# hzyu17/GaussianVI

Measured on AMD Instinct MI355X. Metric: sigma-point psi-evals/sec + NGD iters/sec, 1024-factor d=12 p=5 chain, higher is better.
Workload: dtype f64; 1 GPU; c3: T=1025 states, n=6; 1 step = 1 device-resident NGD iteration; restart every 30; factor_sets_columns=[K factors, d, GH degree p, N sigma points], factor_set_kinds=1024 x quadratic-prior d=12 p=5 (N=17217); 1025 x fixed-prior d=6 p=5 (N=1433), kernel_variant=6, chunks_per_factor=4, fused_pass=True, one_launch_factor_stage=False, mirror_pairs=False, fuse_trial=2

## Files before the change

### gaussianvi_amd/_lib.py

```python
from __future__ import annotations

import ctypes as C
import os

HERE = os.path.dirname(os.path.abspath(__file__))
LIB_PATH = os.environ.get("GVI_LIB_PATH") or os.path.join(HERE, "libgvi_hip.so")

c_double_p = C.POINTER(C.c_double)
c_int32_p = C.POINTER(C.c_int32)
c_int8_p = C.POINTER(C.c_int8)
c_void_pp = C.POINTER(C.c_void_p)
ALLGATHER_FN = C.CFUNCTYPE(C.c_int, C.c_void_p, C.c_void_p, C.c_void_p, C.c_int64, C.c_void_p)

SIGNATURES = {
    "gvi_ctx_create": [C.c_int, C.c_int, c_void_pp],
    "gvi_ctx_destroy": [C.c_void_p],
    "gvi_ctx_set_stream": [C.c_void_p, C.c_void_p],
    "gvi_ctx_sync": [C.c_void_p],
    "gvi_spgh_count": [C.c_int, C.c_int, C.POINTER(C.c_int64)],
    "gvi_spgh_nodes": [C.c_int, C.c_int, C.c_int64, C.c_void_p, C.c_void_p, C.c_void_p],
    "gvi_chain_set": [C.c_void_p, C.c_int, C.c_int],
    "gvi_factors_add": [C.c_void_p, C.c_int, C.c_int, C.c_int, C.c_void_p, C.c_int, C.c_void_p, C.c_int64,
                        C.c_void_p, C.POINTER(C.c_int)],
    "gvi_factors_add_table": [C.c_void_p, C.c_int, C.c_int, C.c_int, C.c_void_p, C.c_int, C.c_void_p, C.c_int64,
# ... 16 lines not shown
    "gvi_prox_step": [C.c_void_p, C.c_double, C.c_int, C.c_void_p, C.c_void_p, C.c_void_p, C.c_void_p],
    "gvi_factors_set_closed_form": [C.c_void_p, C.c_int, C.c_int],
    "gvi_factors_set_sdf3d": [C.c_void_p, C.c_int, C.c_void_p, C.c_double, C.c_int, C.c_int, C.c_int, C.c_void_p],
    "gvi_factors_set_arm": [C.c_void_p, C.c_int, C.c_int, C.c_void_p, C.c_void_p, C.c_void_p, C.c_void_p, C.c_int, C.c_void_p,
                            C.c_void_p, C.c_void_p],
    "gvi_factors_set_temperature": [C.c_void_p, C.c_int, C.c_void_p],
    "gvi_factors_info": [C.c_void_p, C.c_int, C.POINTER(C.c_int), C.POINTER(C.c_int), C.POINTER(C.c_int),
                         C.POINTER(C.c_int64)],
    "gvi_moments": [C.c_void_p, C.c_int] + [C.c_void_p] * 5,
    "gvi_moments_dev": [C.c_void_p, C.c_int] + [C.c_void_p] * 5,
    "gvi_raw_moments": [C.c_void_p, C.c_int] + [C.c_void_p] * 5,
    "gvi_costs": [C.c_void_p, C.c_int] + [C.c_void_p] * 3,
    "gvi_costs_dev": [C.c_void_p, C.c_int] + [C.c_void_p] * 3,
    "gvi_expand": [C.c_void_p, C.c_int] + [C.c_void_p] * 3,
    "gvi_moments_from_psi": [C.c_void_p, C.c_int] + [C.c_void_p] * 6,
    "gvi_bt_assemble": [C.c_void_p, C.c_int, C.c_void_p, C.c_void_p, C.c_void_p, C.c_void_p, C.c_void_p, C.c_void_p],
    "gvi_bt_solve": [C.c_void_p] + [C.c_void_p] * 4,
    "gvi_bt_logdet": [C.c_void_p] + [C.c_void_p] * 3,
    "gvi_bt_marginals": [C.c_void_p] + [C.c_void_p] * 4,
    "gvi_gather_marginals": [C.c_void_p, C.c_int] + [C.c_void_p] * 5,
    "gvi_ngd_init": [C.c_void_p] + [C.c_void_p] * 3,
    "gvi_ngd_cost": [C.c_void_p, c_double_p],
    "gvi_ngd_factor_costs": [C.c_void_p, C.c_int, C.c_void_p],
    "gvi_ngd_gradients": [C.c_void_p],
    "gvi_ngd_trial": [C.c_void_p, C.c_double, c_double_p],
    "gvi_ngd_accept": [C.c_void_p],
    "gvi_ngd_step": [C.c_void_p, C.c_double, C.c_int, c_double_p, C.POINTER(C.c_int), c_double_p, C.POINTER(C.c_int)],
    "gvi_ngd_run": [C.c_void_p, C.c_int, C.c_double, C.c_int, C.c_void_p, C.c_void_p, C.c_void_p, C.c_void_p, C.POINTER(C.c_int)],
    "gvi_ngd_set_mode": [C.c_void_p, C.c_int, C.c_int],
    "gvi_ngd_counters": [C.c_void_p, C.POINTER(C.c_int64), C.POINTER(C.c_int64), C.c_int],
    "gvi_ngd_gradients_local": [C.c_void_p],
    "gvi_ngd_gradients_finish": [C.c_void_p],
    "gvi_ngd_cost_local": [C.c_void_p],
    "gvi_ngd_cost_finish": [C.c_void_p, c_double_p],
    "gvi_ngd_trial_local": [C.c_void_p, C.c_double],
    "gvi_ngd_trial_finish": [C.c_void_p, c_double_p],
    "gvi_ngd_exchange": [C.c_void_p, C.c_int, c_void_pp, C.POINTER(C.c_int64)],
    "gvi_dist_unique_id": [C.c_void_p],
    "gvi_dist_init_rccl": [C.c_void_p, C.c_int, C.c_int, C.c_void_p],
    "gvi_dist_init_callback": [C.c_void_p, C.c_int, C.c_int, C.c_void_p, C.c_void_p],
    "gvi_dist_info": [C.c_void_p, C.POINTER(C.c_int), C.POINTER(C.c_int), C.POINTER(C.c_int)],
    "gvi_ngd_get_state": [C.c_void_p] + [C.c_void_p] * 5,
    "gvi_ngd_get_gradients": [C.c_void_p] + [C.c_void_p] * 6,
    "gvi_randn": [C.c_void_p, C.c_uint64, C.c_int64, C.c_int64, C.c_void_p],
    "gvi_bt_sample": [C.c_void_p, C.c_void_p, C.c_void_p, C.c_void_p, C.c_int, C.c_uint64, C.c_int64, C.c_void_p, C.c_void_p],
    "gvi_ngd_sample": [C.c_void_p, C.c_int, C.c_uint64, C.c_int64, C.c_void_p],
# ... 47 lines not shown
```

### gaussianvi_amd/api.py

```python
from __future__ import annotations

import ctypes as C

import numpy as np

from . import _lib

PSI_RANGE_1D, PSI_QUAD_PRIOR, PSI_FIXED_PRIOR, PSI_HOST_CALLBACK, PSI_HINGE_SDF_2D = 0, 1, 2, 3, 4
PSI_HINGE_SDF_2D_BODY, PSI_HINGE_SDF_3D, PSI_HINGE_SDF_3D_ARM = 5, 6, 7
RULE_NGD, RULE_PROX_JKO = 0, 1
GVI_F64, GVI_F32 = 0, 1


class GviError(RuntimeError):
    def __init__(self, status, msg):
        super().__init__(f"gvi status {status}: {msg}")
        self.status = status


def _f64(a):
    return np.ascontiguousarray(a, dtype=np.float64)


def _p(a):
# ... 212 lines not shown
        return SD, SU

    def gather_marginals(self, sid, mu, SigD, SigU):
        K, d, _, _ = self.sets[sid]
        mu, SigD, SigU = _f64(mu), _f64(SigD), _f64(SigU)
        mk, Sk = np.empty((K, d)), np.empty((K, d, d))
        self._ck(self.lib.gvi_gather_marginals(self.h, sid, _p(mu), _p(SigD), _p(SigU), _p(mk), _p(Sk)))
        return mk, Sk

    def ngd_init(self, mu, D, U):
        mu, D, U = _f64(mu), _f64(D), _f64(U)
        self._ck(self.lib.gvi_ngd_init(self.h, _p(mu), _p(D), _p(U)))

    def ngd_cost(self):
        v = C.c_double()
        self._ck(self.lib.gvi_ngd_cost(self.h, C.byref(v)))
        return v.value

    def ngd_factor_costs(self, sid):
        out = np.empty(self.sets[sid][0])
        self._ck(self.lib.gvi_ngd_factor_costs(self.h, sid, _p(out)))
        return out

    def ngd_gradients(self):
        self._ck(self.lib.gvi_ngd_gradients(self.h))

    def ngd_gradients_local(self):
        self._ck(self.lib.gvi_ngd_gradients_local(self.h))

    def ngd_gradients_finish(self):
        self._ck(self.lib.gvi_ngd_gradients_finish(self.h))

    def ngd_cost_local(self):
        self._ck(self.lib.gvi_ngd_cost_local(self.h))

    def ngd_cost_finish(self):
        v = C.c_double()
        self._ck(self.lib.gvi_ngd_cost_finish(self.h, C.byref(v)))
        return v.value

    def ngd_trial(self, step):
        v = C.c_double()
        self._ck(self.lib.gvi_ngd_trial(self.h, step, C.byref(v)))
        return v.value

    def ngd_trial_local(self, step):
# ... 190 lines not shown
```

### gaussianvi_amd/csrc/gvi_hip.hip

```cpp
#include "../../include/gvi_hip.h"

#include <hip/hip_runtime.h>
#include <hip/hip_ext.h>
#include <dlfcn.h>

#include <algorithm>
#include <chrono>
#include <cassert>
#include <cmath>
#include <cstdio>
#include <cstdlib>
#include <cstring>
#include <memory>
#include <map>
#include <set>
#include <string>
#include <thread>
#include <vector>

#include "host_linalg.hpp"
#include "kernels_bt.hpp"
#include "chain_launch.hpp"
#include "kernels_factor.hpp"
#include "kernels_orbit.hpp"
// ... 129 lines not shown
  int T = 0, n = 0;
  std::vector<std::unique_ptr<FactorSet>> sets;
  std::vector<std::shared_ptr<Table>> tables;
  NgdState ngd;
  DevMem Wbuf, Ibuf, vbuf, scratch, hldtmp;
  std::string err;
  int variant = 0;
  bool warm_start = true;
  int fuse_trial = 2;
  bool last_first_accepted = true;
  int64_t n_full_pass = 0, n_cost_pass = 0;
  bool speculate = true;
  bool profile = false;
  bool profile_all = false;
  int profile_every = 1;
  long profile_count = 0;
  int target_waves = 2048;
  bool mirror = true;
  int split_flush = SPLIT_FLUSH;
  bool sreg_pipe = true;
  bool no_scost = false;
  bool orbit = true;
  bool fused = true;
  int orbit_waves = 4096;
  double jacobi_tol = 1e-34;
  bool prefer_opsi = false;
  bool chol_sqrt = true;
  bool trust_table_degree = false;
  int orbit_min_tiles = 6;
  bool orbit_stack = true;
  int orbit_copies = 8;
  static constexpr int cost_chunk_mult = 8;
  static constexpr int scost_f = 2;
  struct Deferred { int kind = -1; MomArgs a; dim3 grid; int d = 0, m = 0; OrbitArgs oa; int smax = 0; bool all_pos = false; bool capture_any = false; };
  Deferred* defer = nullptr;
  int update_rule = 0;
  bool pair_fuse = true;
  bool defer_gather = false;
  bool fuse_gather = true;
  hipEvent_t fork = nullptr;
  bool side_solve = true;
  hipStream_t side = nullptr;
  hipEvent_t ev_grad = nullptr, ev_solve[2] = {nullptr, nullptr};
  bool solve_pending[2] = {false, false};
  bool dual_chain = true;
  bool solve_deferred[2] = {false, false};
  bool asm_on_load = true;
  bool asm_pending[2] = {false, false};
  DevMem Wbuf2, Ibuf2;
  DevMem chain_sync;
  unsigned chain_seq = 0;
  bool chain_merge = true;
// ... 568 lines not shown

gvi_status run_moments(gvi_ctx* c, FactorSet& s, const double* mu, const double* psi_ext, int full,
                       hipStream_t st = nullptr) {
  if (!st) st = c->stream;
  if (s.K == 0) { s.nchunk = 1; s.chunk = s.table->Np; s.use_reg = s.use_split = s.use_orbit = s.use_opsi = false; return GVI_OK; }
  if (s.kind == KIND_HINGE_SDF_3D_ARM && !psi_ext && !s.arm.p)
    return fail(c, GVI_ERR_STATE, "HINGE_SDF_3D_ARM set without an arm model: call gvi_factors_set_arm");
  if (s.kind >= KIND_HINGE_SDF_2D && !psi_ext && s.sdf_rows == 0)
    return fail(c, GVI_ERR_STATE, "HINGE_SDF set without a grid: call gvi_factors_set_sdf2d / gvi_factors_set_sdf3d");
  bool reg = reg_supported(s.kind, s.d, s.m) && !psi_ext && c->variant != 1;
  if (c->variant == 2 && !reg && !psi_ext)
    return fail(c, GVI_ERR_UNSUPPORTED, "register kernel not instantiated for this (kind, d)");
  const bool closed = s.closed_form && !psi_ext;
  const bool orbit = !closed && !psi_ext && orbit_supported(c, s);
  const bool opsi = !closed && !orbit && !psi_ext && orbit_psi_supported(c, s, reg);
  const bool split = !closed && !orbit && !opsi && !reg && !psi_ext && c->variant != 1 && split_supported(s);
  if (closed) { reg = false; s.chunk = s.table->Np; s.nchunk = 1; }
  else if (orbit || opsi) {
    reg = false;
    const int64_t tiles = (int64_t)s.table->orb.tile_s.size();
    const int64_t by_waves = std::max<int64_t>(1, (c->orbit_waves + s.K - 1) / s.K);
    const int64_t by_tiles = std::max<int64_t>(1, tiles / std::max(1, c->orbit_min_tiles));
    s.nchunk = (int)std::min<int64_t>(tiles, std::min(by_waves, by_tiles));
    s.chunk = s.table->Np;
  } else if (split) {
    const int64_t tiles = s.table->Np / 64;
    int64_t nch = std::max<int64_t>(1, (1024 + s.K - 1) / s.K);
    nch = std::max<int64_t>(nch, (tiles + 16383) / 16384);
    nch = std::min<int64_t>(nch, tiles);
    s.chunk = (tiles + nch - 1) / nch * 64;
    s.nchunk = (int)((s.table->Np + s.chunk - 1) / s.chunk);
  } else plan_chunks(c, s, reg);
  if (reg && !full && !closed && !orbit && (c->variant == 5 || c->variant == 0) && scost_supported(s) && !c->no_scost) {
    const int64_t iters = s.table->Np / 256;
    int64_t nch = std::min<int64_t>(std::max<int64_t>(1, (int64_t)s.nchunk * c->cost_chunk_mult), std::max<int64_t>(1, iters));
    const int64_t per = (iters + nch - 1) / nch;
    s.chunk = per * 256;
    s.nchunk = (int)((s.table->Np + s.chunk - 1) / s.chunk);
  }
  s.use_reg = reg;
  s.use_split = split;
  s.use_orbit = orbit;
  s.use_opsi = opsi;
  const size_t need = (size_t)s.K * s.nchunk * npairs(s.d) * 8;
  HIPCK(c, s.partial.ensure(need));
  MomArgs a;
// ... 196 lines not shown

const char* gvi_version(void) { return "gvi_hip 0.1 (gfx950, fp64)"; }

const char* gvi_last_error(const gvi_ctx* ctx) { return ctx ? ctx->err.c_str() : g_noctx_err.c_str(); }

gvi_status gvi_ctx_create(int device, int dtype, gvi_ctx** out) {
  if (!out) return fail(nullptr, GVI_ERR_ARG, "out is NULL");
  *out = nullptr;
  if (dtype == GVI_F32) return fail(nullptr, GVI_ERR_UNSUPPORTED, "GVI_F32 (config 5) is not implemented yet");
  if (dtype != GVI_F64) return fail(nullptr, GVI_ERR_ARG, "unknown dtype");
  int ndev = 0;
  hipError_t e = hipGetDeviceCount(&ndev);
  if (e != hipSuccess || ndev <= 0)
    return fail(nullptr, GVI_ERR_HIP, "no HIP device: this library has no CPU fallback");
  if (device < 0 || device >= ndev) return fail(nullptr, GVI_ERR_ARG, "device index out of range");
  if (hipSetDevice(device) != hipSuccess) return fail(nullptr, GVI_ERR_HIP, "hipSetDevice failed");
  std::unique_ptr<gvi_ctx> c(new gvi_ctx);
  c->device = device; c->dtype = dtype;
  if (hipStreamCreateWithFlags(&c->stream, hipStreamNonBlocking) != hipSuccess)
    return fail(nullptr, GVI_ERR_HIP, "hipStreamCreate failed");
  if (const char* w = getenv("GVI_NO_SCOST")) c->no_scost = atoi(w) != 0;
  if (const char* w = getenv("GVI_ORBIT")) c->orbit = atoi(w) != 0;
  if (const char* w = getenv("GVI_FUSED")) c->fused = atoi(w) != 0;
  if (const char* w = getenv("GVI_ASM_ON_LOAD")) c->asm_on_load = atoi(w) != 0;
  if (const char* w = getenv("GVI_PIPELINE")) c->pipeline = atoi(w) != 0;
  if (const char* w = getenv("GVI_CHAIN_WAVE")) chain_wave_enabled() = atoi(w) != 0;
  if (const char* w = getenv("GVI_ASM_DENSE")) chain_asm_dense_enabled() = atoi(w) != 0;
  if (const char* w = getenv("GVI_CHAIN_MERGE")) c->chain_merge = atoi(w) != 0;
  if (const char* w = getenv("GVI_SREG_PIPE")) c->sreg_pipe = atoi(w) != 0;
  if (const char* w = getenv("GVI_MIRROR")) c->mirror = atoi(w) != 0;
  if (const char* w = getenv("GVI_NO_PAIR")) c->pair_fuse = atoi(w) == 0;
  if (const char* w = getenv("GVI_NO_FUSE_GATHER")) c->fuse_gather = atoi(w) == 0;
  if (const char* w = getenv("GVI_SIDE_SOLVE")) c->side_solve = atoi(w) != 0;
  if (const char* w = getenv("GVI_FUSE_TRIAL")) c->fuse_trial = std::min(2, std::max(0, atoi(w)));
  if (const char* w = getenv("GVI_SPIN_MS")) c->spin_ms = std::max(0, atoi(w));
  if (const char* w = getenv("GVI_SAFE_PUBLISH")) c->safe_publish = atoi(w) != 0;
  if (hipEventCreateWithFlags(&c->fork, hipEventDisableTiming) != hipSuccess ||
      hipHostMalloc((void**)&c->host_slot, 128, hipHostMallocMapped | hipHostMallocCoherent) != hipSuccess ||
      hipHostGetDevicePointer((void**)&c->host_slot_dev, c->host_slot, 0) != hipSuccess)
    return fail(nullptr, GVI_ERR_HIP, "event / host-mapped slot allocation failed");
  for (int q = 0; q < 16; ++q) c->host_slot[q] = 0.0;
  *out = c.release();
  return GVI_OK;
}

gvi_status gvi_ctx_destroy(gvi_ctx* ctx) {
// ... 1001 lines not shown
}

gvi_status gvi_ngd_cost_local(gvi_ctx* ctx) {
  GVICK(ngd_check(ctx));
  HIPCK(ctx, hipSetDevice(ctx->device));
  return ngd_cost_local(ctx, ctx->ngd.cur);
}

gvi_status gvi_ngd_cost_finish(gvi_ctx* ctx, double* cost) {
  GVICK(ngd_check(ctx));
  HIPCK(ctx, hipSetDevice(ctx->device));
  return ngd_cost_finish(ctx, ctx->ngd.cur, cost);
}

gvi_status gvi_ngd_factor_costs(gvi_ctx* ctx, int set_id, double* costs) {
  GVICK(ngd_check(ctx));
  FactorSet* s = get_set(ctx, set_id);
  if (!s || !costs) return fail(ctx, GVI_ERR_ARG, "bad set id / NULL");
  HIPCK(ctx, hipSetDevice(ctx->device));
  const int i = ctx->ngd.cur;
  GVICK(ngd_flush_gather(ctx, i));
  GVICK(gvi_costs_dev(ctx, set_id, s->mu_k[i].d(), s->Sigma_k[i].d(), s->cost.d()));
  GVICK(d2h(ctx, costs, s->cost.p, (size_t)s->K * 8));
  return sync(ctx);
}

static gvi_status ngd_moments_launch(gvi_ctx* ctx, int slot, int full) {
  if (full) ++ctx->n_full_pass; else ++ctx->n_cost_pass;
  if (ctx->pair_fuse && ctx->sets.size() == 2 && !ctx->profile_all) {
    FactorSet& s0 = *ctx->sets[0];
    FactorSet& s1 = *ctx->sets[1];
    const bool shape = s0.kind == KIND_QUAD_PRIOR && s1.kind == KIND_FIXED_PRIOR && s0.d == 12 && s1.d == 6 &&
                       !s0.closed_form && !s1.closed_form && s0.K > 0 && s1.K > 0;
    const bool shape_orbit = orbit_supported(ctx, s0) && orbit_supported(ctx, s1) && s0.m == s1.m && s0.all_pos && s1.all_pos &&
                             !s0.closed_form && !s1.closed_form && s0.K > 0 && s1.K > 0;
    if (shape || shape_orbit) {
      gvi_ctx::Deferred d0, d1;
      ctx->defer = &d0;
      gvi_status st = run_moments(ctx, s0, s0.mu_k[slot].d(), nullptr, full);
      if (st == GVI_OK) { ctx->defer = &d1; st = run_moments(ctx, s1, s1.mu_k[slot].d(), nullptr, full); }
      ctx->defer = nullptr;
      GVICK(st);
      const int want = full ? 0 : 1;
      if (d0.kind == 2 && d1.kind == 2) {
        const bool prof = ctx->profile && full && (ctx->profile_count++ % ctx->profile_every) == 0;
        if (prof) {
// ... 97 lines not shown
  if (ctx->update_rule != GVI_RULE_NGD) return false;
  const int m = ctx->sets[0]->m;
  for (auto& sp : ctx->sets) {
    const FactorSet& s = *sp;
    if (!orbit_supported(ctx, s) || !s.all_pos || s.closed_form || s.K <= 0 || s.m != m) return false;
    if (s.prep_slot == slot) return false;
    if (s.table->orb.tile_s.empty()) return false;
  }
  const int d0 = ctx->sets[0]->d, d1 = ctx->sets.size() > 1 ? ctx->sets[1]->d : d0 / 2;
  if (!((m == 6 && d0 == 12 && d1 == 6) || (m == 2 && d0 == 4 && d1 == 2))) return false;
  for (auto& sp : ctx->sets)
    if (!sp->dev().chol) return false;
  return fused_nblk(ctx) > 0;
}

static gvi_status ngd_fused_full(gvi_ctx* ctx, int slot, int publish_slot) {
  NgdState& g = ctx->ngd;
  FusedArgs A{};
  A.nsets = (int)ctx->sets.size();
  A.koff[0] = 0;
  int smax = 0, dmax = 0, copies = 1;
  const int m = ctx->sets[0]->m;
  A.nblk = fused_nblk(ctx);
  for (int si = 0; si < A.nsets; ++si) {
    FactorSet& s = *ctx->sets[si];
    FusedSet& F = A.s[si];
    s.prep_slot = -1;
    s.nchunk = 4; s.chunk = s.table->Np;
    s.use_reg = s.use_split = false; s.use_orbit = true; s.fused_pair = true;
    F.f = s.dev();
    if (ctx->warm_start) {
      if (s.Vws.bytes == 0) { HIPCK(ctx, s.Vws.ensure((size_t)s.K * s.d * s.d * 8)); s.warm_count = 0; }
      F.f.Vws = s.Vws.d();
      F.f.warm = (s.warm_count % 32) != 0;
      s.warm_count++;
    }
    GVICK(orbit_args(ctx, s, 1, &F.oa));
    F.oa.partial = nullptr;
    F.mu = s.mu_k[slot].d(); F.Sigma = s.Sigma_k[slot].d();
    F.start = s.chain_structured ? nullptr : (const int32_t*)s.dstart.p;
    F.mu_k = s.mu_k[slot].d(); F.Sigma_k = s.Sigma_k[slot].d();
    F.Ephi = s.Ephi.d(); F.cost = s.cost.d(); F.Vdmu = s.Vdmu.d(); F.Vddmu = s.Vddmu.d();
    A.koff[si + 1] = A.koff[si] + s.K;
    A.cl.cost[si] = s.cost.d(); A.cl.K[si] = s.K;
    smax = std::max(smax, s.table->orb.smax);
    dmax = std::max(dmax, s.d);
// ... 1002 lines not shown
  if (!s) return GVI_ERR_ARG;
  if (variant) *variant = s->closed_form ? 0 : (s->use_opsi ? 7 : s->use_orbit ? 6 : (s->fused_pair ? 5 : (s->use_reg ? 2 : (s->use_split ? 3 : 1))));
  if (nchunk) *nchunk = s->nchunk;
  if (chunk) *chunk = s->chunk;
  return GVI_OK;
}

gvi_status gvi_set_option(gvi_ctx* ctx, const char* name, int value) {
  if (!ctx || !name) return GVI_ERR_ARG;
  const std::string n(name);
  if (ctx->ngd.ready) { GVICK(ngd_flush_assemble(ctx, 0)); GVICK(ngd_flush_assemble(ctx, 1)); }
  if (n == "split_flush") ctx->split_flush = std::max(0, value);
  else if (n == "sreg_pipe") ctx->sreg_pipe = value != 0;
  else if (n == "mirror") ctx->mirror = value != 0;
  else if (n == "pair_fuse") ctx->pair_fuse = value != 0;
  else if (n == "fuse_gather") ctx->fuse_gather = value != 0;
  else if (n == "side_solve") ctx->side_solve = value != 0;
  else if (n == "dual_chain") ctx->dual_chain = value != 0;
  else if (n == "warm_start") ctx->warm_start = value != 0;
  else if (n == "no_scost") ctx->no_scost = value != 0;
  else if (n == "target_waves") ctx->target_waves = std::max(1, value);
  else if (n == "orbit") ctx->orbit = value != 0;
  else if (n == "fused") ctx->fused = value != 0;
  else if (n == "assemble_on_load") ctx->asm_on_load = value != 0;
  else if (n == "pipeline") ctx->pipeline = value != 0;
  else if (n == "chain_wave") chain_wave_enabled() = value != 0;
  else if (n == "asm_dense") chain_asm_dense_enabled() = value != 0;
  else if (n == "sample_sweep") ctx->sample_sweep = value != 0;
  else if (n == "chain_merge") { ctx->chain_merge = value != 0; ctx->chain_merge_fault = value == 2; }
  else if (n == "trust_table_degree") ctx->trust_table_degree = value != 0;
  else if (n == "safe_publish") {
    GVICK(sync(ctx));
    ctx->safe_publish = value != 0;
    for (int q = 0; q < 16; ++q) ctx->host_slot[q] = 0.0;
  }
  else if (n == "chol_sqrt") { ctx->chol_sqrt = value != 0; for (auto& s : ctx->sets) s->use_chol = ctx->chol_sqrt; }
  else if (n == "jacobi_tol_exp") {
    if (value > -20) return fail(ctx, GVI_ERR_ARG, "jacobi_tol_exp must be <= -20 (threshold 10^value on squared magnitudes)");
    ctx->jacobi_tol = std::pow(10.0, (double)value);
    for (auto& s : ctx->sets) s->jtol = ctx->jacobi_tol;
  }
  else if (n == "orbit_waves") ctx->orbit_waves = std::max(1, value);
  else if (n == "orbit_min_tiles") ctx->orbit_min_tiles = std::max(1, value);
  else if (n == "orbit_stack") ctx->orbit_stack = value != 0;
  else if (n == "orbit_copies") ctx->orbit_copies = std::min(16, std::max(1, value));
  else return fail(ctx, GVI_ERR_ARG, "unknown option: " + n);
  for (auto& s : ctx->sets) s->prep_slot = -1;
  ctx->ngd.cost_valid[0] = ctx->ngd.cost_valid[1] = false;
  ctx->ngd.grad_valid = false;
  ctx->ngd.spec_ready = false;
  return GVI_OK;
}


gvi_status gvi_debug_cost_log(gvi_ctx* ctx, int entries, double* out, double* seq_now) {
  if (!ctx) return GVI_ERR_ARG;
  HIPCK(ctx, hipSetDevice(ctx->device));
  GVICK(sync(ctx));
  if (entries > 0) {
    if (entries & (entries - 1)) return fail(ctx, GVI_ERR_ARG, "entries must be a power of two");
    HIPCK(ctx, ctx->dbg_log.ensure((size_t)entries * 8));
    HIPCK(ctx, hipMemset(ctx->dbg_log.p, 0, (size_t)entries * 8));
    ctx->dbg_mask = entries - 1;
    double* lg = ctx->dbg_log.d();
    HIPCK(ctx, hipMemcpyToSymbol(HIP_SYMBOL(gvi_dbg_mask), &ctx->dbg_mask, sizeof(int)));
    HIPCK(ctx, hipMemcpyToSymbol(HIP_SYMBOL(gvi_dbg_log), &lg, sizeof(double*)));
// ... 178 lines not shown
```

### gaussianvi_amd/csrc/kernels_factor.hpp

```cpp
#pragma once
#include <hip/hip_runtime.h>
#include <stdint.h>

#include <utility>

#include "device_common.hpp"

namespace gvi {

enum { KIND_RANGE_1D = 0, KIND_QUAD_PRIOR = 1, KIND_FIXED_PRIOR = 2, KIND_HOST_CALLBACK = 3, KIND_HINGE_SDF_2D = 4,
       KIND_HINGE_SDF_2D_BODY = 5, KIND_HINGE_SDF_3D = 6, KIND_HINGE_SDF_3D_ARM = 7 };

__host__ __device__ inline int npairs(int d) { return (d + 1) * (d + 2) / 2; }

__host__ __device__ inline int pair_index(int d, int a, int b) {
  return 1 + d + a * d - a * (a - 1) / 2 + (b - a);
}

struct FactorDev {
  int K, d, m, kind;
  int64_t N, Np;
  const double* Zt;
  const double* w;
  const double* Zq;
// ... 1676 lines not shown
__global__ __launch_bounds__(256) void moments_scost_pair_kernel(MomArgs a0, MomArgs a1, int nbx0, int nb0, int nbx1) {
  if (pred_skip(a0.pred, a0.pred_val)) return;
  constexpr int MM = M0 > M1 ? M0 : M1;
  __shared__ double us[4 * F * 3 * MM];
  const int b = blockIdx.x;
  if (b < nb0) scost_body<D0, M0, F>(a0, b % nbx0, b / nbx0, us);
  else scost_body<D1, M1, F>(a1, (b - nb0) % nbx1, (b - nb0) / nbx1, us);
}

struct EpiArgs {
  FactorDev f;
  const double* partial;
  int nchunk, full;
  double* Ephi;
  double* cost;
  double* Vdmu;
  double* Vddmu;
  double* E_xmuphi;
  double* E_xxphi;
};

__host__ __device__ inline size_t epilogue_lds_doubles(int d) { return (size_t)npairs(d) + 4 * (size_t)d * d; }

template <int DT>
__device__ __forceinline__ double epilogue_body_t(const EpiArgs& a, int k, double* sm, int phase, const double* P, double* Zs = nullptr) {
  const FactorDev& f = a.f;
  const int d = DT ? DT : f.d, dd = d * d, lane = threadIdx.x & 63;
  const int npo = a.full ? npairs(d) : 1;
  double* Ms = sm;
  double* M2 = Ms + npairs(d);
  double* Tm = M2 + dd;
  double* Sv = Zs ? Zs : Tm + dd;
  double* Lv = Tm + 2 * dd;
  const double Tk = f.temperature[k];
  const bool want_v = a.full && (a.Vdmu || a.Vddmu);
  if (want_v && phase != 2 && !Zs) {
    const double* Sinv = f.Sinv + (size_t)k * dd;
    const double* Lam = f.Lam + (size_t)k * dd;
    for (int e = lane; e < dd; e += 64) { Sv[e] = Sinv[e]; Lv[e] = Lam[e]; }
  }
  for (int j = lane; j < npo && phase != 2; j += 64) {
    double s = 0.0;
    for (int c0 = 0; c0 < a.nchunk; c0 += 8) {
      double pv[8];
#pragma unroll
      for (int q = 0; q < 8; ++q) pv[q] = c0 + q < a.nchunk ? P[(size_t)(c0 + q) * npo + j] : 0.0;
#pragma unroll
      for (int q = 0; q < 8; ++q) s += pv[q];
    }
    Ms[j] = s;
// ... 159 lines not shown
struct EpiTail {
  int on;
  double* acc;
  const double* half_logdet;
  double* host_out;
  double seq;
  unsigned* counter;
  const double* pred;
  double pred_val;
  double* accept;
  double* cost_dev;
  int slot_cur, slot_trial;
  int c0_use_imm;
  double c0_imm;
  int safe;
};

struct CostList {
  int nsets;
  double* cost[MAX_FSETS];
  int K[MAX_FSETS];
};

__device__ __forceinline__ void epi_tail_arrive(const CostList& cl, const EpiTail& tail, double* cost_slot, const double costk, const int lane,
                                                const unsigned bid, const unsigned nblocks, int* last) {
  if (lane == 0) {
    __hip_atomic_store(cost_slot, costk, __ATOMIC_RELAXED, __HIP_MEMORY_SCOPE_AGENT);
    asm volatile("s_waitcnt vmcnt(0)" ::: "memory");
    const unsigned grp = bid / EPI_GROUP, ngrp = (nblocks + EPI_GROUP - 1) / EPI_GROUP;
    const unsigned in_grp = grp + 1 < ngrp ? (unsigned)EPI_GROUP : nblocks - grp * EPI_GROUP;
    unsigned* gc = tail.counter + 32u * (1u + grp);
    int l = 0;
    const bool lastg = tail.safe ? __hip_atomic_fetch_add(gc, 1u, __ATOMIC_ACQ_REL, __HIP_MEMORY_SCOPE_AGENT) == in_grp - 1
                                 : __hip_atomic_fetch_add(gc, 1u, __ATOMIC_RELAXED, __HIP_MEMORY_SCOPE_AGENT) == in_grp - 1;
    if (lastg) {
      __hip_atomic_store(gc, 0u, __ATOMIC_RELAXED, __HIP_MEMORY_SCOPE_AGENT);
      l = ngrp == 1 ? 1
                    : (tail.safe ? __hip_atomic_fetch_add(tail.counter, 1u, __ATOMIC_ACQ_REL, __HIP_MEMORY_SCOPE_AGENT) == ngrp - 1
                                 : __hip_atomic_fetch_add(tail.counter, 1u, __ATOMIC_RELAXED, __HIP_MEMORY_SCOPE_AGENT) == ngrp - 1);
    }
    *last = l;
  }
  wave_lds_sync();
  if (!*last) return;
  double total = 0.0;
  for (int s2 = 0; s2 < cl.nsets; ++s2) {
    const double* cost = cl.cost[s2];
    const int K = cl.K[s2];
    double p[4][8];
#pragma unroll
    for (int j = 0; j < 4; ++j)
#pragma unroll
      for (int q = 0; q < 8; ++q) {
        const int k = lane + 64 * j + q * 256;
        p[j][q] = k < K ? __hip_atomic_load(cost + k, __ATOMIC_RELAXED, __HIP_MEMORY_SCOPE_AGENT) : 0.0;
      }
    double vs[4];
#pragma unroll
    for (int j = 0; j < 4; ++j) {
      double s = 0.0;
#pragma unroll
      for (int q = 0; q < 8; ++q) s += p[j][q];
      for (int k0 = lane + 64 * j + 8 * 256; k0 < K; k0 += 8 * 256) {
        double pp[8];
#pragma unroll
        for (int q = 0; q < 8; ++q) {
          const int k = k0 + q * 256;
          pp[q] = k < K ? __hip_atomic_load(cost + k, __ATOMIC_RELAXED, __HIP_MEMORY_SCOPE_AGENT) : 0.0;
        }
#pragma unroll
        for (int q = 0; q < 8; ++q) s += pp[q];
      }
      vs[j] = s;
    }
    double t = (vs[0] + vs[2]) + (vs[1] + vs[3]);
#pragma unroll
    for (int w = 32; w > 0; w >>= 1) t += __shfl_down(t, w);
// ... 44 lines not shown
```

### gaussianvi_amd/csrc/kernels_fused.hpp

```cpp
#pragma once
#include "kernels_orbit.hpp"

namespace gvi {

constexpr int FUSED_MAX_ITEMS = 4;

struct FusedSet {
  FactorDev f;
  OrbitArgs oa;
  const double* mu;
  const double* Sigma;
  const int32_t* start;
  double* mu_k;
  double* Sigma_k;
  double* Ephi;
  double* cost;
  double* Vdmu;
  double* Vddmu;
};

struct FusedArgs {
  int nsets;
  int nblk;
  int koff[3];
  FusedSet s[2];
  int gather, n;
  const double* gmu;
  const double* gdmu;
  double gstep;
  const double* SigD;
  const double* SigU;
  double* mu_out;
  int64_t nmu;
  EpiTail tail;
  CostList cl;
};

__host__ __device__ inline size_t fused_item_doubles(int d) {
  const size_t dd = (size_t)d * d, dp = d + (d & 1);
  const size_t prep = 4 * dd + 2 * dp + 3 * d + (dp + 1) / 2 + 1 + dd + d + 2;
  const size_t epi = epilogue_lds_doubles(d) + 2;
  return ((prep > epi ? prep : epi) + 1) & ~(size_t)1;
}
__host__ __device__ inline size_t fused_region_doubles(int dmax, int M, int copies) {
  const size_t a = (size_t)orbit_lds_doubles(dmax, M, copies), b = fused_item_doubles(dmax);
  return ((a > b ? a : b) + 1) & ~(size_t)1;
}
// ... 66 lines not shown
  constexpr int KA_LINES = (sizeof(FusedArgs) + 3 * 8 + 63) / 64;
  static_assert(KA_LINES == 26, "kernarg_warm: one specialisation per argument block size");
  kernarg_warm<KA_LINES>();
  PREP_STAMP(11);
  asm volatile("" :: "s"(pred_p), "s"(nblk_), "s"(K0), "s"(K1_), "s"(nsets_));
  PREP_STAMP(12);
  const LazyPred lpred = pred_issue(pred_p, A.tail.pred_val);
  const int wave = __builtin_amdgcn_readfirstlane(threadIdx.x >> 6);
  const int b = (int)blockIdx.x;
  if (b >= nblk_) {
    const int64_t j = (int64_t)(b - A.nblk) * 256 + threadIdx.x;
    const double v = j < A.nmu ? A.gmu[j] + A.gstep * A.gdmu[j] : 0.0;
    if (pred_fail(lpred)) return;
    if (j < A.nmu) A.mu_out[j] = v;
    return;
  }
  const int K1 = nsets_ > 1 ? K1_ : 0;
  int c0 = 0, c1 = 0;
#pragma unroll
  for (int j = 0; j < FUSED_MAX_ITEMS; ++j) { c0 += b + j * nblk_ < K0; c1 += b + j * nblk_ < K1; }
  const int nitems = c0 + c1;
  __shared__ int hw_simd[4];
  __shared__ int l_ready[FUSED_MAX_ITEMS];
  const int simd = (int)__builtin_amdgcn_s_getreg((1 << 11) | (4 << 6) | 4);
  const int slot = (int)__builtin_amdgcn_s_getreg((3 << 11) | (0 << 6) | 4);
  if ((threadIdx.x & 63) == 0) { hw_simd[wave] = simd | (slot << 4); l_ready[wave] = 0; }
  __syncthreads();
  PREP_STAMP(13);
  const int h0 = hw_simd[0], h1 = hw_simd[1], h2 = hw_simd[2], h3 = hw_simd[3];
  const bool spread = ((1 << (h0 & 3)) | (1 << (h1 & 3)) | (1 << (h2 & 3)) | (1 << (h3 & 3))) == 15;
  const int iw = __builtin_amdgcn_readfirstlane(spread ? (simd - (h0 >> 4)) & 3 : wave);
  const size_t region = fused_region_doubles(dmax, M, copies_max);
  double* Zbase = sm + 4 * region;
  const size_t zs = fused_keep_doubles(dmax, M), ps = (size_t)4 * npairs(dmax);
  const size_t oH = (size_t)dmax * dmax, oU = oH + (size_t)dmax * orbit_hstride(M);
  double* Pbase = Zbase + (size_t)maxitems * zs;
  const int nhelp = min(4 - nitems, nitems);
  const auto helped = [&](const int it) {
    const FactorDev& f = A.s[it < c0 ? 0 : 1].f;
    return it < nhelp && f.m > 0 && f.m * f.d <= 128;
  };
  if (iw < nitems) {
    const int si = iw < c0 ? 0 : 1;
    const int k = b + (iw < c0 ? iw : iw - c0) * A.nblk;
    const FusedSet& S = A.s[si];
    const FactorDev& f = S.f;
    const int d = f.d, dd = d * d, lane = threadIdx.x & 63;
    double* area = sm + (size_t)wave * region;
    double* Zs = Zbase + (size_t)iw * zs;
// ... 22 lines not shown
      for (int w = 0; w < 4; ++w) {
        const int hw = w == 0 ? h0 : (w == 1 ? h1 : (w == 2 ? h2 : h3));
        if ((((hw & 3) - (h0 >> 4)) & 3) == it) wi = w;
      }
    }
    double* own = sm + (size_t)wave * region;
    double* Zs = Zbase + (size_t)it * zs;
    double* mh = own + (size_t)S.f.m * d;
    if (lane < d) {
      double mval;
      if (A.gather) {
        const size_t j = (size_t)(S.start ? S.start[k] : k) * A.n + lane;
        mval = A.gdmu ? A.gmu[j] + A.gstep * A.gdmu[j] : A.gmu[j];
      } else mval = S.mu[(size_t)k * d + lane];
      mh[lane] = mval;
    }
    if (!pred_fail(lpred)) {
      if (si == 0) prep_chol_hu0<D0>(S.f, mh, k, own, sm + (size_t)wi * region, &l_ready[it], Zs + oH, Zs + oU, orbit_hstride(M));
      else prep_chol_hu0<D1>(S.f, mh, k, own, sm + (size_t)wi * region, &l_ready[it], Zs + oH, Zs + oU, orbit_hstride(M));
    }
  }
  FUSED_STAMP(1);
  if (pred_fail(lpred)) return;
  __syncthreads();
  FUSED_STAMP(2);
  for (int it = 0; it < nitems; ++it) {
    const int si = it < c0 ? 0 : 1;
    const int k = b + (it < c0 ? it : it - c0) * A.nblk;
    const FusedSet& S = A.s[si];
    const double* Zi = Zbase + (size_t)it * zs;
    orbit_wave<M, SMAX, true, false, true>(S.oa, k, wave, sm + (size_t)wave * region, Pbase + (size_t)it * ps + (size_t)wave * npairs(S.f.d),
                                           Zi + oH, Zi + oU);
  }
  FUSED_STAMP(3);
  __syncthreads();
  FUSED_STAMP(4);
  const bool helpers = A.tail.on && nitems <= 2;
  if (iw >= nitems) {
    const int it = iw - 2;
    if (!helpers || it < 0 || it >= nitems) return;
    const int si = it < c0 ? 0 : 1;
    const int k = b + (it < c0 ? it : it - c0) * A.nblk;
    const FusedSet& S = A.s[si];
    const double Tk = S.f.temperature[k];
    const double* Pl = Pbase + (size_t)it * ps;
    const int npo = npairs(S.f.d);
    double m0 = 0.0;
#pragma unroll
    for (int q = 0; q < 4; ++q) m0 += Pl[(size_t)q * npo];
    const double costk = m0 / Tk;
    epi_tail_arrive(A.cl, A.tail, S.cost + k, costk, (int)(threadIdx.x & 63), (unsigned)(A.koff[si] + k), (unsigned)A.koff[A.nsets],
                    (int*)(sm + (size_t)wave * region));
    return;
  }
  {
    const int si = iw < c0 ? 0 : 1;
    const int k = b + (iw < c0 ? iw : iw - c0) * A.nblk;
    const FusedSet& S = A.s[si];
    const int d = S.f.d;
    double* area = sm + (size_t)wave * region;
    double* Zs = Zbase + (size_t)iw * zs;
    const double* Pl = Pbase + (size_t)iw * ps;
    EpiArgs e;
    e.f = S.f; e.partial = nullptr; e.nchunk = 4; e.full = 1;
    e.Ephi = S.Ephi; e.cost = helpers ? nullptr : S.cost; e.Vdmu = S.Vdmu; e.Vddmu = S.Vddmu; e.E_xmuphi = nullptr; e.E_xxphi = nullptr;
    auto epi = [&](int phase) { return si == 0 ? epilogue_body_t<D0>(e, k, area, phase, Pl, Zs) : epilogue_body_t<D1>(e, k, area, phase, Pl, Zs); };
    if (!A.tail.on || helpers) { epi(0); return; }
    const double costk = epi(1);
    FUSED_STAMP(5);
    int* last = (int*)(area + epilogue_lds_doubles(d));
    epi_tail_arrive(A.cl, A.tail, S.cost + k, costk, (int)(threadIdx.x & 63), (unsigned)(A.koff[si] + k), (unsigned)A.koff[A.nsets], last);
    FUSED_STAMP(6);
    epi(2);
    FUSED_STAMP(7);
  }
}

}
```

### gaussianvi_amd/csrc/kernels_orbit.hpp

```cpp
#pragma once
#include <hip/hip_runtime.h>
#include <stdint.h>

#include "kernels_factor.hpp"

namespace gvi {

#ifdef GVI_FUSED_TIMING
__device__ unsigned long long* gvi_walk_stamps;
#endif

struct OrbitDev {
  const uint64_t* cpk;
  const uint64_t* rpk;
  const double* mag;
  const double* w;
  const int32_t* bounds;
  int64_t norb_p;
  double w0;
  int32_t cend[8];
  int32_t bnd[5];
  int32_t nb;
  int32_t cbase[8], cgrp[8], cstride[8];
};
// ... 503 lines not shown
    if constexpr (!PIPE) orbit_load<S>(ob, cb8 + (uint32_t)t * 512u, cur);
    const int tn = t + 1 < t1 ? t + 1 : t;
    auto pre = [&]() {
      if constexpr (PIPE) {
        __builtin_amdgcn_sched_barrier(0);
        orbit_load<S>(ob, cb8 + (uint32_t)tn * 512u, cur);
        __builtin_amdgcn_sched_barrier(0);
      }
    };
    const uint64_t cpk = cur.cpk, rpk = cur.rpk;
    const double w = cur.w;
    double mg[S];
#pragma unroll
    for (int j = 0; j < S; ++j) mg[j] = cur.mg[j];
    if constexpr (M == 12 && S >= 4 && FULL) orbit_walk_split<S, SIGNED>(lc, cpk, rpk, mg, w, Hl, accl, su0, sg, k0, m0, pre);
    else orbit_walk<M, S, FULL, SIGNED>(lc, cpk, rpk, mg, w, Hl, accl, su0, sg, k0, m0, pre);
  }
}

template <int M, int SMAX, bool FULL, bool SIGNED, bool FRESH = false>
__device__ __forceinline__ void orbit_wave(const OrbitArgs& a, const int k, const int chunk, double* lds, double* out,
                                           const double* Hpre = nullptr, const double* u0pre = nullptr) {
  const OrbitDev& ob = a.ob;
  const int lane = threadIdx.x & 63, d = a.d;
#ifdef GVI_FUSED_TIMING
  const long long wt_start = clock64();
#endif
  const int NP = FULL ? (d + 1) * (d + 2) / 2 : 1;
  int tb, te;
  if (ob.nb) { tb = ob.bnd[chunk]; te = ob.bnd[chunk + 1]; }
  else { tb = ob.bounds[chunk]; te = ob.bounds[chunk + 1]; }
  tb = __builtin_amdgcn_readfirstlane(tb);
  te = __builtin_amdgcn_readfirstlane(te);
  const uint32_t lane8 = (uint32_t)lane * 8u;
  const double* Hl = Hpre ? Hpre : lds;
  const int C = a.copies, lc = __builtin_ctz((unsigned)C);
  double* accl = lds + d * orbit_hstride(M);
  if (!Hpre) {
    const double* Hg = a.H + (size_t)k * M * d;
    for (int e = lane; e < d * M; e += 64) lds[(e / M) * orbit_hstride(M) + e % M] = Hg[e];
  }
  if (FULL)
    for (int e = lane; e < NP * C; e += 64) accl[e] = 0.0;
  double* accme = accl + (lane & (C - 1));
  double su0[M], sg[M], k0 = 0.0;
#pragma unroll
  for (int r = 0; r < M; ++r) {
// ... 125 lines not shown
```

### include/gvi_hip.h

```cpp
#ifndef GVI_HIP_H
#define GVI_HIP_H

#include <stdint.h>

#ifdef __cplusplus
extern "C" {
#endif

typedef struct gvi_ctx gvi_ctx;
typedef int gvi_status;

enum {
  GVI_OK = 0,
  GVI_ERR_ARG = 1,
  GVI_ERR_HIP = 2,
  GVI_ERR_UNSUPPORTED = 3,
  GVI_ERR_NOTABLE = 4,
  GVI_ERR_STATE = 5
};
enum { GVI_F64 = 0, GVI_F32 = 1 };

enum { GVI_PSI_RANGE_1D = 0, GVI_PSI_QUAD_PRIOR = 1, GVI_PSI_FIXED_PRIOR = 2, GVI_PSI_HOST_CALLBACK = 3,
       GVI_PSI_HINGE_SDF_2D = 4, GVI_PSI_HINGE_SDF_2D_BODY = 5, GVI_PSI_HINGE_SDF_3D = 6, GVI_PSI_HINGE_SDF_3D_ARM = 7 };

// ... 35 lines not shown
gvi_status gvi_moments(gvi_ctx* ctx, int set_id, const double* mu, const double* Sigma,
                       double* Ephi, double* Vdmu, double* Vddmu);
gvi_status gvi_moments_dev(gvi_ctx* ctx, int set_id, const double* mu, const double* Sigma,
                           double* Ephi, double* Vdmu, double* Vddmu);
gvi_status gvi_raw_moments(gvi_ctx* ctx, int set_id, const double* mu, const double* Sigma,
                           double* E_phi, double* E_xmuphi, double* E_xxphi);
gvi_status gvi_costs(gvi_ctx* ctx, int set_id, const double* mu, const double* Sigma, double* cost);
gvi_status gvi_costs_dev(gvi_ctx* ctx, int set_id, const double* mu, const double* Sigma, double* cost);
gvi_status gvi_expand(gvi_ctx* ctx, int set_id, const double* mu, const double* Sigma, double* X);
gvi_status gvi_moments_from_psi(gvi_ctx* ctx, int set_id, const double* mu, const double* Sigma,
                                const double* psi, double* Ephi, double* Vdmu, double* Vddmu);

gvi_status gvi_bt_assemble(gvi_ctx* ctx, int nsets, const int* set_ids, const double* const* Vdmu,
                           const double* const* Vddmu, double* g, double* D, double* U);
gvi_status gvi_bt_solve(gvi_ctx* ctx, const double* D, const double* U, const double* rhs, double* x);
gvi_status gvi_bt_logdet(gvi_ctx* ctx, const double* D, const double* U, double* half_logdet);
gvi_status gvi_bt_marginals(gvi_ctx* ctx, const double* D, const double* U, double* SigD, double* SigU);
gvi_status gvi_gather_marginals(gvi_ctx* ctx, int set_id, const double* mu, const double* SigD,
                                const double* SigU, double* mu_k, double* Sigma_k);

gvi_status gvi_ngd_init(gvi_ctx* ctx, const double* mu, const double* D, const double* U);
gvi_status gvi_ngd_cost(gvi_ctx* ctx, double* cost);
gvi_status gvi_ngd_factor_costs(gvi_ctx* ctx, int set_id, double* costs);
gvi_status gvi_ngd_gradients(gvi_ctx* ctx);
gvi_status gvi_ngd_trial(gvi_ctx* ctx, double step, double* new_cost);
gvi_status gvi_ngd_accept(gvi_ctx* ctx);
gvi_status gvi_ngd_step(gvi_ctx* ctx, double step_size_base, int max_backtrack, double* cost_iter,
                        int* accepted, double* new_cost, int* ntrials);
gvi_status gvi_ngd_run(gvi_ctx* ctx, int max_iters, double step_size_base, int max_backtrack, double* cost_iter,
                       int* accepted, double* new_cost, int* ntrials, int* iters_done);
gvi_status gvi_ngd_set_mode(gvi_ctx* ctx, int speculate, int fuse_trial);
gvi_status gvi_ngd_counters(gvi_ctx* ctx, int64_t* full_passes, int64_t* cost_passes, int reset);

enum { GVI_RULE_NGD = 0, GVI_RULE_PROX_JKO = 1 };
gvi_status gvi_ngd_set_update_rule(gvi_ctx* ctx, int rule);
gvi_status gvi_prox_gradients(gvi_ctx* ctx, double h);
gvi_status gvi_prox_trial(gvi_ctx* ctx, double step, double* new_cost);
gvi_status gvi_prox_step(gvi_ctx* ctx, double step_size_base, int max_backtrack, double* cost_iter, int* decreased,
                         double* new_cost, int* ntrials);
gvi_status gvi_ngd_gradients_local(gvi_ctx* ctx);
gvi_status gvi_ngd_gradients_finish(gvi_ctx* ctx);
gvi_status gvi_ngd_cost_local(gvi_ctx* ctx);
gvi_status gvi_ngd_cost_finish(gvi_ctx* ctx, double* cost);
gvi_status gvi_ngd_trial_local(gvi_ctx* ctx, double step);
gvi_status gvi_ngd_trial_finish(gvi_ctx* ctx, double* new_cost);
gvi_status gvi_ngd_exchange(gvi_ctx* ctx, int which, void** dev_ptr, int64_t* count);
// ... 37 lines not shown
```

Before: 210.3 billion psi-evals/s.

## Overlap early orbit chunks with epilogue in fused factor kernel

Adds a fused_overlap mode, on by default. When a block holds one item from each set and helper waves exist, the waves split differently: waves 1 and 3 compute the second item's orbit chunks early and coordinate through LDS flags instead of block-wide barriers, so one item's epilogue can overlap with the other's orbit work. It also pins lane IDs through asm barriers to steer register allocation, adds an orbit_chunks override, and adds a debug getter for factor moments. The risks are spin-wait overhead, a possible deadlock if the wave roles are wrong, and extra complexity in the control flow.

```diff
diff --git a/gaussianvi_amd/_lib.py b/gaussianvi_amd/_lib.py
--- a/gaussianvi_amd/_lib.py
+++ b/gaussianvi_amd/_lib.py
@@ -62,6 +62,7 @@
     "gvi_ngd_init": [C.c_void_p] + [C.c_void_p] * 3,
     "gvi_ngd_cost": [C.c_void_p, c_double_p],
     "gvi_ngd_factor_costs": [C.c_void_p, C.c_int, C.c_void_p],
+    "gvi_ngd_factor_moments": [C.c_void_p, C.c_int] + [C.c_void_p] * 4,
     "gvi_ngd_gradients": [C.c_void_p],
     "gvi_ngd_trial": [C.c_void_p, C.c_double, c_double_p],
     "gvi_ngd_accept": [C.c_void_p],
diff --git a/gaussianvi_amd/api.py b/gaussianvi_amd/api.py
--- a/gaussianvi_amd/api.py
+++ b/gaussianvi_amd/api.py
@@ -258,6 +258,12 @@
         self._ck(self.lib.gvi_ngd_factor_costs(self.h, sid, _p(out)))
         return out
 
+    def ngd_factor_moments(self, sid):
+        K, d, _, _ = self.sets[sid]
+        out = dict(Ephi=np.empty(K), cost=np.empty(K), Vdmu=np.empty((K, d)), Vddmu=np.empty((K, d, d)))
+        self._ck(self.lib.gvi_ngd_factor_moments(self.h, sid, *[_p(out[k]) for k in ("Ephi", "cost", "Vdmu", "Vddmu")]))
+        return out
+
     def ngd_gradients(self):
         self._ck(self.lib.gvi_ngd_gradients(self.h))
 
diff --git a/gaussianvi_amd/csrc/gvi_hip.hip b/gaussianvi_amd/csrc/gvi_hip.hip
--- a/gaussianvi_amd/csrc/gvi_hip.hip
+++ b/gaussianvi_amd/csrc/gvi_hip.hip
@@ -175,12 +175,14 @@
   bool no_scost = false;
   bool orbit = true;
   bool fused = true;
+  int fused_overlap = 1;
   int orbit_waves = 4096;
   double jacobi_tol = 1e-34;
   bool prefer_opsi = false;
   bool chol_sqrt = true;
   bool trust_table_degree = false;
   int orbit_min_tiles = 6;
+  int orbit_chunks = 0;
   bool orbit_stack = true;
   int orbit_copies = 8;
   static constexpr int cost_chunk_mult = 8;
@@ -795,6 +797,7 @@
     const int64_t by_waves = std::max<int64_t>(1, (c->orbit_waves + s.K - 1) / s.K);
     const int64_t by_tiles = std::max<int64_t>(1, tiles / std::max(1, c->orbit_min_tiles));
     s.nchunk = (int)std::min<int64_t>(tiles, std::min(by_waves, by_tiles));
+    if (c->orbit_chunks > 0 && full) s.nchunk = (int)std::min<int64_t>(tiles, c->orbit_chunks);
     s.chunk = s.table->Np;
   } else if (split) {
     const int64_t tiles = s.table->Np / 64;
@@ -1037,6 +1040,7 @@
   if (const char* w = getenv("GVI_NO_SCOST")) c->no_scost = atoi(w) != 0;
   if (const char* w = getenv("GVI_ORBIT")) c->orbit = atoi(w) != 0;
   if (const char* w = getenv("GVI_FUSED")) c->fused = atoi(w) != 0;
+  if (const char* w = getenv("GVI_FUSED_OVERLAP")) c->fused_overlap = std::min(3, std::max(0, atoi(w)));
   if (const char* w = getenv("GVI_ASM_ON_LOAD")) c->asm_on_load = atoi(w) != 0;
   if (const char* w = getenv("GVI_PIPELINE")) c->pipeline = atoi(w) != 0;
   if (const char* w = getenv("GVI_CHAIN_WAVE")) chain_wave_enabled() = atoi(w) != 0;
@@ -2084,6 +2088,19 @@
   GVICK(ngd_flush_gather(ctx, i));
   GVICK(gvi_costs_dev(ctx, set_id, s->mu_k[i].d(), s->Sigma_k[i].d(), s->cost.d()));
   GVICK(d2h(ctx, costs, s->cost.p, (size_t)s->K * 8));
+  return sync(ctx);
+}
+
+gvi_status gvi_ngd_factor_moments(gvi_ctx* ctx, int set_id, double* Ephi, double* cost, double* Vdmu, double* Vddmu) {
+  GVICK(ngd_check(ctx));
+  FactorSet* s = get_set(ctx, set_id);
+  if (!s) return fail(ctx, GVI_ERR_ARG, "bad set id");
+  HIPCK(ctx, hipSetDevice(ctx->device));
+  const size_t K = (size_t)s->K, d = (size_t)s->d;
+  if (Ephi) GVICK(d2h(ctx, Ephi, s->Ephi.p, K * 8));
+  if (cost) GVICK(d2h(ctx, cost, s->cost.p, K * 8));
+  if (Vdmu) GVICK(d2h(ctx, Vdmu, s->Vdmu.p, K * d * 8));
+  if (Vddmu) GVICK(d2h(ctx, Vddmu, s->Vddmu.p, K * d * d * 8));
   return sync(ctx);
 }
 
@@ -2227,6 +2244,7 @@
   int smax = 0, dmax = 0, copies = 1;
   const int m = ctx->sets[0]->m;
   A.nblk = fused_nblk(ctx);
+  A.overlap = ctx->fused_overlap;
   for (int si = 0; si < A.nsets; ++si) {
     FactorSet& s = *ctx->sets[si];
     FusedSet& F = A.s[si];
@@ -3275,6 +3293,10 @@
   else if (n == "target_waves") ctx->target_waves = std::max(1, value);
   else if (n == "orbit") ctx->orbit = value != 0;
   else if (n == "fused") ctx->fused = value != 0;
+  else if (n == "fused_overlap") {
+    if (value < 0 || value > 3) return fail(ctx, GVI_ERR_ARG, "fused_overlap: 0 .. 3");
+    ctx->fused_overlap = value;
+  }
   else if (n == "assemble_on_load") ctx->asm_on_load = value != 0;
   else if (n == "pipeline") ctx->pipeline = value != 0;
   else if (n == "chain_wave") chain_wave_enabled() = value != 0;
@@ -3295,6 +3317,7 @@
   }
   else if (n == "orbit_waves") ctx->orbit_waves = std::max(1, value);
   else if (n == "orbit_min_tiles") ctx->orbit_min_tiles = std::max(1, value);
+  else if (n == "orbit_chunks") ctx->orbit_chunks = std::max(0, value);
   else if (n == "orbit_stack") ctx->orbit_stack = value != 0;
   else if (n == "orbit_copies") ctx->orbit_copies = std::min(16, std::max(1, value));
   else return fail(ctx, GVI_ERR_ARG, "unknown option: " + n);
diff --git a/gaussianvi_amd/csrc/kernels_factor.hpp b/gaussianvi_amd/csrc/kernels_factor.hpp
--- a/gaussianvi_amd/csrc/kernels_factor.hpp
+++ b/gaussianvi_amd/csrc/kernels_factor.hpp
@@ -1722,10 +1722,15 @@
 
 __host__ __device__ inline size_t epilogue_lds_doubles(int d) { return (size_t)npairs(d) + 4 * (size_t)d * d; }
 
-template <int DT>
+template <int DT, bool INLOOP = false>
 __device__ __forceinline__ double epilogue_body_t(const EpiArgs& a, int k, double* sm, int phase, const double* P, double* Zs = nullptr) {
   const FactorDev& f = a.f;
-  const int d = DT ? DT : f.d, dd = d * d, lane = threadIdx.x & 63;
+  const int d = DT ? DT : f.d, dd = d * d;
+  int lane = threadIdx.x & 63;
+  if constexpr (INLOOP) {
+    lane = (int)__lane_id();
+    asm volatile("" : "+v"(lane));
+  }
   const int npo = a.full ? npairs(d) : 1;
   double* Ms = sm;
   double* M2 = Ms + npairs(d);
@@ -1931,6 +1936,7 @@
   int K[MAX_FSETS];
 };
 
+template <bool LEAN = false>
 __device__ __forceinline__ void epi_tail_arrive(const CostList& cl, const EpiTail& tail, double* cost_slot, const double costk, const int lane,
                                                 const unsigned bid, const unsigned nblocks, int* last) {
   if (lane == 0) {
@@ -1956,12 +1962,14 @@
   for (int s2 = 0; s2 < cl.nsets; ++s2) {
     const double* cost = cl.cost[s2];
     const int K = cl.K[s2];
+    int ln = lane;
+    if constexpr (LEAN) asm volatile("" : "+v"(ln));
     double p[4][8];
 #pragma unroll
     for (int j = 0; j < 4; ++j)
 #pragma unroll
       for (int q = 0; q < 8; ++q) {
-        const int k = lane + 64 * j + q * 256;
+        const int k = ln + 64 * j + q * 256;
         p[j][q] = k < K ? __hip_atomic_load(cost + k, __ATOMIC_RELAXED, __HIP_MEMORY_SCOPE_AGENT) : 0.0;
       }
     double vs[4];
diff --git a/gaussianvi_amd/csrc/kernels_fused.hpp b/gaussianvi_amd/csrc/kernels_fused.hpp
--- a/gaussianvi_amd/csrc/kernels_fused.hpp
+++ b/gaussianvi_amd/csrc/kernels_fused.hpp
@@ -23,6 +23,7 @@
   int nsets;
   int nblk;
   int koff[3];
+  int overlap;
   FusedSet s[2];
   int gather, n;
   const double* gmu;
@@ -135,9 +136,10 @@
   const int nitems = c0 + c1;
   __shared__ int hw_simd[4];
   __shared__ int l_ready[FUSED_MAX_ITEMS];
+  __shared__ int l_early[2];
   const int simd = (int)__builtin_amdgcn_s_getreg((1 << 11) | (4 << 6) | 4);
   const int slot = (int)__builtin_amdgcn_s_getreg((3 << 11) | (0 << 6) | 4);
-  if ((threadIdx.x & 63) == 0) { hw_simd[wave] = simd | (slot << 4); l_ready[wave] = 0; }
+  if ((threadIdx.x & 63) == 0) { hw_simd[wave] = simd | (slot << 4); l_ready[wave] = 0; l_early[wave & 1] = 0; }
   __syncthreads();
   PREP_STAMP(13);
   const int h0 = hw_simd[0], h1 = hw_simd[1], h2 = hw_simd[2], h3 = hw_simd[3];
@@ -206,58 +208,89 @@
   }
   FUSED_STAMP(1);
   if (pred_fail(lpred)) return;
-  __syncthreads();
-  FUSED_STAMP(2);
-  for (int it = 0; it < nitems; ++it) {
-    const int si = it < c0 ? 0 : 1;
-    const int k = b + (it < c0 ? it : it - c0) * A.nblk;
-    const FusedSet& S = A.s[si];
-    const double* Zi = Zbase + (size_t)it * zs;
-    orbit_wave<M, SMAX, true, false, true>(S.oa, k, wave, sm + (size_t)wave * region, Pbase + (size_t)it * ps + (size_t)wave * npairs(S.f.d),
-                                           Zi + oH, Zi + oU);
-  }
-  FUSED_STAMP(3);
-  __syncthreads();
-  FUSED_STAMP(4);
-  const bool helpers = A.tail.on && nitems <= 2;
-  if (iw >= nitems) {
-    const int it = iw - 2;
-    if (!helpers || it < 0 || it >= nitems) return;
-    const int si = it < c0 ? 0 : 1;
-    const int k = b + (it < c0 ? it : it - c0) * A.nblk;
-    const FusedSet& S = A.s[si];
-    const double Tk = S.f.temperature[k];
-    const double* Pl = Pbase + (size_t)it * ps;
-    const int npo = npairs(S.f.d);
-    double m0 = 0.0;
-#pragma unroll
-    for (int q = 0; q < 4; ++q) m0 += Pl[(size_t)q * npo];
-    const double costk = m0 / Tk;
-    epi_tail_arrive(A.cl, A.tail, S.cost + k, costk, (int)(threadIdx.x & 63), (unsigned)(A.koff[si] + k), (unsigned)A.koff[A.nsets],
-                    (int*)(sm + (size_t)wave * region));
-    return;
-  }
-  {
-    const int si = iw < c0 ? 0 : 1;
-    const int k = b + (iw < c0 ? iw : iw - c0) * A.nblk;
+  const bool early = (A.overlap & 1) && nitems == 2 && c0 == 1 && helped(1);
+  int st = early ? 0 : 1;
+  asm volatile("" : "+v"(st));
+  st = __builtin_amdgcn_readfirstlane(st);
+  for (;; ++st) {
+    if (st) {
+      __syncthreads();
+      FUSED_STAMP(2);
+    } else if (iw == 3) {
+      wave_lds_sync();
+      if (__lane_id() == 0) __hip_atomic_store(&l_early[0], 1, __ATOMIC_RELAXED, __HIP_MEMORY_SCOPE_WORKGROUP);
+    } else if (iw == 1) {
+      while (__hip_atomic_load(&l_early[0], __ATOMIC_RELAXED, __HIP_MEMORY_SCOPE_WORKGROUP) == 0) __builtin_amdgcn_s_sleep(1);
+      asm volatile("" ::: "memory");
+    }
+    const int njobs = st ? (early ? 1 : nitems) : ((iw & 1) ? 2 : 0);
+    for (int j = 0; j < njobs; ++j) {
+      const int it = st ? j : 1, chunk = st ? wave : (iw & 2) + j;
+      const int si = it < c0 ? 0 : 1;
+      const int k = b + (it < c0 ? it : it - c0) * A.nblk;
+      const FusedSet& S = A.s[si];
+      const double* Zi = Zbase + (size_t)it * zs;
+      orbit_wave<M, SMAX, true, false, true>(S.oa, k, chunk, sm + (size_t)wave * region, Pbase + (size_t)it * ps + (size_t)chunk * npairs(S.f.d),
+                                             Zi + oH, Zi + oU);
+    }
+    if (st) {
+      FUSED_STAMP(3);
+      __syncthreads();
+      FUSED_STAMP(4);
+    } else if (iw == 3) {
+      wave_lds_sync();
+      if (__lane_id() == 0) __hip_atomic_store(&l_early[1], 1, __ATOMIC_RELAXED, __HIP_MEMORY_SCOPE_WORKGROUP);
+      continue;
+    } else if (iw == 1) {
+      while (__hip_atomic_load(&l_early[1], __ATOMIC_RELAXED, __HIP_MEMORY_SCOPE_WORKGROUP) == 0) __builtin_amdgcn_s_sleep(1);
+      asm volatile("" ::: "memory");
+    } else continue;
+    int iwq = iw;
+    asm volatile("" : "+s"(iwq));
+    const bool helpers = A.tail.on && nitems <= 2;
+    if (iwq >= nitems) {
+      const int it = iwq - 2;
+      if (!helpers || it < 0 || it >= nitems) return;
+      const int si = it < c0 ? 0 : 1;
+      const int k = b + (it < c0 ? it : it - c0) * A.nblk;
+      const FusedSet& S = A.s[si];
+      const double Tk = S.f.temperature[k];
+      const double* Pl = Pbase + (size_t)it * ps;
+      const int npo = npairs(S.f.d);
+      double m0 = 0.0;
+#pragma unroll
+      for (int q = 0; q < 4; ++q) m0 += Pl[(size_t)q * npo];
+      const double costk = m0 / Tk;
+      epi_tail_arrive<true>(A.cl, A.tail, S.cost + k, costk, (int)__lane_id(), (unsigned)(A.koff[si] + k), (unsigned)A.koff[A.nsets],
+                      (int*)(sm + (size_t)wave * region));
+      return;
+    }
+    if (st && early && iwq == 1) return;
+    const int si = iwq < c0 ? 0 : 1;
+    const int k = b + (iwq < c0 ? iwq : iwq - c0) * A.nblk;
     const FusedSet& S = A.s[si];
     const int d = S.f.d;
     double* area = sm + (size_t)wave * region;
-    double* Zs = Zbase + (size_t)iw * zs;
-    const double* Pl = Pbase + (size_t)iw * ps;
+    double* Zs = Zbase + (size_t)iwq * zs;
+    const double* Pl = Pbase + (size_t)iwq * ps;
     EpiArgs e;
     e.f = S.f; e.partial = nullptr; e.nchunk = 4; e.full = 1;
     e.Ephi = S.Ephi; e.cost = helpers ? nullptr : S.cost; e.Vdmu = S.Vdmu; e.Vddmu = S.Vddmu; e.E_xmuphi = nullptr; e.E_xxphi = nullptr;
-    auto epi = [&](int phase) { return si == 0 ? epilogue_body_t<D0>(e, k, area, phase, Pl, Zs) : epilogue_body_t<D1>(e, k, area, phase, Pl, Zs); };
-    if (!A.tail.on || helpers) { epi(0); return; }
+    auto epi = [&](int phase) { return si == 0 ? epilogue_body_t<D0, true>(e, k, area, phase, Pl, Zs) : epilogue_body_t<D1, true>(e, k, area, phase, Pl, Zs); };
+    if (!A.tail.on || helpers) {
+      epi(0);
+      if (st) return;
+      continue;
+    }
     const double costk = epi(1);
     FUSED_STAMP(5);
     int* last = (int*)(area + epilogue_lds_doubles(d));
-    epi_tail_arrive(A.cl, A.tail, S.cost + k, costk, (int)(threadIdx.x & 63), (unsigned)(A.koff[si] + k), (unsigned)A.koff[A.nsets], last);
+    epi_tail_arrive<true>(A.cl, A.tail, S.cost + k, costk, (int)__lane_id(), (unsigned)(A.koff[si] + k), (unsigned)A.koff[A.nsets], last);
     FUSED_STAMP(6);
     epi(2);
     FUSED_STAMP(7);
-  }
-}
-
-}
+    return;
+  }
+}
+
+}
diff --git a/gaussianvi_amd/csrc/kernels_orbit.hpp b/gaussianvi_amd/csrc/kernels_orbit.hpp
--- a/gaussianvi_amd/csrc/kernels_orbit.hpp
+++ b/gaussianvi_amd/csrc/kernels_orbit.hpp
@@ -549,7 +549,9 @@
 __device__ __forceinline__ void orbit_wave(const OrbitArgs& a, const int k, const int chunk, double* lds, double* out,
                                            const double* Hpre = nullptr, const double* u0pre = nullptr) {
   const OrbitDev& ob = a.ob;
-  const int lane = threadIdx.x & 63, d = a.d;
+  const int d = a.d;
+  int lane = (int)__lane_id();
+  asm volatile("" : "+v"(lane));
 #ifdef GVI_FUSED_TIMING
   const long long wt_start = clock64();
 #endif
diff --git a/include/gvi_hip.h b/include/gvi_hip.h
--- a/include/gvi_hip.h
+++ b/include/gvi_hip.h
@@ -81,6 +81,7 @@
 gvi_status gvi_ngd_init(gvi_ctx* ctx, const double* mu, const double* D, const double* U);
 gvi_status gvi_ngd_cost(gvi_ctx* ctx, double* cost);
 gvi_status gvi_ngd_factor_costs(gvi_ctx* ctx, int set_id, double* costs);
+gvi_status gvi_ngd_factor_moments(gvi_ctx* ctx, int set_id, double* Ephi, double* cost, double* Vdmu, double* Vddmu);
 gvi_status gvi_ngd_gradients(gvi_ctx* ctx);
 gvi_status gvi_ngd_trial(gvi_ctx* ctx, double step, double* new_cost);
 gvi_status gvi_ngd_accept(gvi_ctx* ctx);
```

Result: slower. 204.8 billion psi-evals/s (-2.6%).
